# Lagrange-Labs/mapreduce-plonky2

Measured on AMD Instinct MI355X. Metric: leaf proofs/sec (whole node) + NTT GB/s vs HBM peak, 2^20-row table build, 1/2/4/8 GPU, higher is better.
Workload: dtype u64 (Goldilocks field)

## Files before the change

mapreduce-plonky2_amd/csrc/gl.cuh:

```cuda
#pragma once
#include <hip/hip_runtime.h>
#include <stdint.h>

typedef uint64_t u64;
typedef uint32_t u32;

#define GL_P 0xFFFFFFFF00000001ULL
#define GL_EPS 0xFFFFFFFFULL
#define GL_MULT_GEN 14293326489335486720ULL
#define GL_TWO_GEN 7277203076849721926ULL

#define GLD __device__ __forceinline__
#define GLHD __host__ __device__ __forceinline__

GLHD u64 gl_mk(u32 lo, u32 hi) { return ((u64)hi << 32) | lo; }
GLHD u64 gl_canon(u64 a) {
  u32 c0, c1;
  u32 t0 = __builtin_addc((u32)a, 0xFFFFFFFFu, 0u, &c0);
  u32 t1 = __builtin_addc((u32)(a >> 32), 0u, c0, &c1);
  return c1 ? gl_mk(t0, t1) : a;
}
GLHD u64 gl_add(u64 a, u64 b) {
  u32 c0, c1, d0, d1;
  u32 s0 = __builtin_addc((u32)a, (u32)b, 0u, &c0);
// ... 5 lines not shown
GLHD u64 gl_sub(u64 a, u64 b) {
  u32 c0, c1, d0, d1;
  u32 s0 = __builtin_subc((u32)a, (u32)b, 0u, &c0);
  u32 s1 = __builtin_subc((u32)(a >> 32), (u32)(b >> 32), c0, &c1);
  u32 m = c1 ? 0xFFFFFFFFu : 0u;
  u32 t0 = __builtin_subc(s0, m, 0u, &d0);
  u32 t1 = __builtin_subc(s1, 0u, d0, &d1);
  return gl_mk(t0, t1);
}
GLHD u64 gl_neg(u64 a) { return a ? GL_P - a : 0; }
GLHD u64 gl_dbl(u64 a) { return gl_add(a, a); }

GLHD u64 gl_addw(u64 a, u64 b) {
  u32 c0, c1;
  u32 s0 = __builtin_addc((u32)a, (u32)b, 0u, &c0);
  u32 s1 = __builtin_addc((u32)(a >> 32), (u32)(b >> 32), c0, &c1);
#if defined(__HIP_DEVICE_COMPILE__)
  return gl_mk(s0, s1) + (u64)(c1 ? 0xFFFFFFFFu : 0u);
#else
  u32 m = c1 ? 0xFFFFFFFFu : 0u, d0, d1;
  u32 t0 = __builtin_addc(s0, m, 0u, &d0);
  u32 t1 = __builtin_addc(s1, 0u, d0, &d1);
  return gl_mk(t0, t1);
#endif
}
GLHD u64 gl_reduce128w(u64 lo, u64 hi) {
#if defined(__HIP_DEVICE_COMPILE__)
  u32 hl = (u32)hi, hh = (u32)(hi >> 32);
  u64 t, c;
  asm("v_mad_u64_u32 %0, %1, %2, -1, %3" : "=&v"(t), "=s"(c) : "v"(hl), "v"(lo));
  u32 t0 = (u32)t, t1 = (u32)(t >> 32), r0, r1, mb, mc;
  asm("v_sub_co_u32 %0, vcc, %4, %6\n\t"
      "v_subbrev_co_u32 %1, vcc, 0, %5, vcc\n\t"
      "v_subb_co_u32 %2, vcc, %0, %0, vcc\n\t"
      "v_cndmask_b32 %3, 0, -1, %7"
      : "=&v"(r0), "=&v"(r1), "=&v"(mb), "=&v"(mc)
      : "v"(t0), "v"(t1), "v"(hh), "s"(c)
      : "vcc");
  return gl_mk(r0, r1) + gl_mk(mc - mb, mb & ~mc);
#else
  u64 hi_hi = hi >> 32, hi_lo = hi & GL_EPS;
  u64 t0;
  bool b = __builtin_sub_overflow(lo, hi_hi, &t0);
  t0 -= b ? GL_EPS : 0;
  u64 t1 = (hi_lo << 32) - hi_lo;
  u64 r;
// ... 146 lines not shown
```

mapreduce-plonky2_amd/csrc/ntt.h:

```cpp
#pragma once
#include "gl.cuh"
#include <map>
#include <memory>

namespace mp2g {

struct NttPlan {
  u32 log_n = 0, log_n1 = 0, log_n2 = 0;
  u64 *tw_a = nullptr, *tw_b = nullptr, *tw4_lo = nullptr, *tw4_hi = nullptr, *tw4_full = nullptr;
  u64 *tc_a = nullptr, *tc_b = nullptr;
  u64 n_inv = 0;
  ~NttPlan();
};
struct CosetTables {
  u32 log_n = 0, logK = 0;
  u64 shift = 0;
  u64 *lo = nullptr, *hi = nullptr, *full = nullptr;
  ~CosetTables();
};

struct NttEngine {
  hipStream_t stream = nullptr;
  std::map<u32, std::unique_ptr<NttPlan>> plans;
  std::map<u64, std::unique_ptr<CosetTables>> cosets;
  u64* scratch = nullptr;
  size_t scratch_words = 0;
  u64 generation = 0;
  ~NttEngine();

  hipError_t plan(u32 log_n, bool inverse, NttPlan** out);
  hipError_t coset(u32 log_n, u32 logK, u64 shift, CosetTables** out);
  hipError_t ensure_scratch(size_t words);
  hipError_t run(const u64* in, u64* out, u32 log_n, u32 polys, u32 logK, u64 in_poly_stride,
                 u64 out_poly_stride, bool inverse, const CosetTables* pre, bool bitrev_out);
// ... 6 lines not shown
```

mapreduce-plonky2_amd/csrc/ntt.hip:

```cpp
#include "ntt.h"
#include <cstdlib>

namespace mp2g {

__device__ __forceinline__ int lds_pad(int a) { return a + (a >> 4); }

struct NttArgs {
  const u64* in;
  u64* out;
  u64 in_poly_stride, out_poly_stride;
  u32 logK;
  u32 log_n, log_n1, log_n2;
  u32 batch;
  const u64* tw;
  const u64* tw4_lo;
  const u64* tw4_hi;
  const u64* pre_lo;
  const u64* pre_hi;
  const u64* tw4_full;
  const u64* pre_full;
  u64 post;
  u32 bitrev_out;
  u32 inverse;
  const u64* tc;
};

template <int LT, int LW> struct NttGeom {
  static constexpr int E = (1 << LT) << LW;
  static constexpr int NT = (E >> 3) < 64 ? 64 : ((E >> 3) > 1024 ? 1024 : (E >> 3));
};
template <int LT> struct R8Tw {
  static constexpr int lo(int rho) { return LT - 3 - 3 * rho; }
  static constexpr int n_tables() { int r = 0; while (lo(r) >= 1) r++; return r; }
  static constexpr int off(int rho) { int o = 0; for (int q = 0; q < rho; q++) o += 7 << lo(q); return o; }
  static constexpr int TOTAL = off(n_tables());
  static constexpr int GLOBAL_ROUNDS = (LT >= 11 && n_tables() >= 1) ? 1 : 0;
  static constexpr int LDS_OFF = off(GLOBAL_ROUNDS);
  static constexpr int LDS_WORDS = TOTAL - LDS_OFF;
};
__device__ __forceinline__ u64 gl_mul_2p24(u64 x) { return gl_canon(gl_reduce96w(x << 24, x >> 40)); }
__device__ __forceinline__ u64 gl_mul_2p48(u64 x) { return gl_reduce128(x << 48, x >> 16); }
__device__ __forceinline__ u64 gl_mul_2p72(u64 x) {
  return gl_sub(gl_reduce128(0, x << 8), (x >> 56) << 32);
}
template <int K> __device__ __forceinline__ u64 gl_mul_w8(u64 x) {
  return K == 1 ? gl_mul_2p24(x) : (K == 2 ? gl_mul_2p48(x) : gl_mul_2p72(x));
}
__device__ __forceinline__ u64 gl_sub_mul_2p48(u64 u, u64 v) {
  u32 c0, c1;
  const u32 s0 = __builtin_subc((u32)u, (u32)v, 0u, &c0);
  const u32 s1 = __builtin_subc((u32)(u >> 32), (u32)(v >> 32), c0, &c1);
  const u64 s = gl_mk(s0, s1);
  return gl_reduce128(gl_mk(c1 ? 0x10000u : 0u, s0 << 16), s >> 16);
}
__device__ __forceinline__ u64 gl_sub_mul_2p72(u64 u, u64 v) {
  u32 c0, c1;
  const u32 s0 = __builtin_subc((u32)u, (u32)v, 0u, &c0);
  const u32 s1 = __builtin_subc((u32)(u >> 32), (u32)(v >> 32), c0, &c1);
  const u64 s = gl_mk(s0, s1);
  return gl_sub(gl_reduce128(gl_mk(0u, c1 ? 0x100u : 0u), s << 8), (s >> 56) << 32);
}
template <int K> __device__ __forceinline__ u64 gl_sub_mul_w8(u64 u, u64 v) {
  return K == 1 ? gl_mul_2p24(gl_sub(u, v)) : (K == 2 ? gl_sub_mul_2p48(u, v) : gl_sub_mul_2p72(u, v));
}
template <int K> __device__ __forceinline__ u64 bfly_lo(u64 u, u64 v, bool inverse) {
  return inverse ? gl_sub_mul_w8<4 - K>(v, u) : gl_sub_mul_w8<K>(u, v);
}
template <int S> __device__ __forceinline__ u64 gl_mul_2pow(u64 x) {
  static_assert(S >= 0 && S < 192, "exponent mod 192");
  if constexpr (S == 0) return x;
  else if constexpr (S >= 96) return gl_neg(gl_mul_2pow<S - 96>(x));
  else if constexpr (S <= 32) return gl_canon(gl_reduce96w(x << S, x >> (64 - S)));
  else if constexpr (S < 64) return gl_reduce128(x << S, x >> (64 - S));
  else if constexpr (S == 64) return gl_reduce128(0, x);
  else {
    constexpr int K = S - 64;
    return gl_sub(gl_reduce128(0, x << K), (x >> (64 - K)) << 32);
  }
}
template <int A, bool INV, int M> __device__ __forceinline__ u64 shift_tw1(u64 x) {
  constexpr int R = ((M & 1) << 2) | (M & 2) | (M >> 2);
  constexpr int E = (A * R) & 63;
  return gl_mul_2pow<3 * (INV ? (64 - E) & 63 : E)>(x);
}
template <int A, bool INV> __device__ __forceinline__ void shift_tw(u64* x) {
  x[1] = shift_tw1<A, INV, 1>(x[1]); x[2] = shift_tw1<A, INV, 2>(x[2]); x[3] = shift_tw1<A, INV, 3>(x[3]); x[4] = shift_tw1<A, INV, 4>(x[4]);
  x[5] = shift_tw1<A, INV, 5>(x[5]); x[6] = shift_tw1<A, INV, 6>(x[6]); x[7] = shift_tw1<A, INV, 7>(x[7]);
}
template <bool INV> __device__ __forceinline__ void shift_twiddles_dir(u64* x, int a) {
  switch (a) {
    case 1: shift_tw<1, INV>(x); break;
    case 2: shift_tw<2, INV>(x); break;
    case 3: shift_tw<3, INV>(x); break;
    case 4: shift_tw<4, INV>(x); break;
    case 5: shift_tw<5, INV>(x); break;
    case 6: shift_tw<6, INV>(x); break;
    case 7: shift_tw<7, INV>(x); break;
    default: break;
  }
}
__device__ __forceinline__ void shift_twiddles(u64* x, int a, bool inverse) {
  if (inverse) shift_twiddles_dir<true>(x, a); else shift_twiddles_dir<false>(x, a);
}

template <int LT, int HI, int R, bool TWG = false, bool MERGED = false>
__device__ __forceinline__ void butterfly(u64* x, int below, const u64* tw, const u64* __restrict__ twg, bool inverse) {
  constexpr int LO = HI - R + 1;
  constexpr int RHO = (LT - 1 - HI) / 3;
  static_assert(R == 3 || LO == 0, "a partial round can only be the last one");
  if constexpr (R == 3) {
    { u64 u = x[0], v = x[4]; x[0] = gl_add(u, v); x[4] = gl_sub(u, v); }
    { u64 u = x[1], v = x[5]; x[1] = gl_add(u, v); x[5] = bfly_lo<1>(u, v, inverse); }
    { u64 u = x[2], v = x[6]; x[2] = gl_add(u, v); x[6] = bfly_lo<2>(u, v, inverse); }
    { u64 u = x[3], v = x[7]; x[3] = gl_add(u, v); x[7] = bfly_lo<3>(u, v, inverse); }
#pragma unroll
    for (int h = 0; h < 8; h += 4) {
      { u64 u = x[h], v = x[h + 2]; x[h] = gl_add(u, v); x[h + 2] = gl_sub(u, v); }
      { u64 u = x[h + 1], v = x[h + 3]; x[h + 1] = gl_add(u, v); x[h + 3] = bfly_lo<2>(u, v, inverse); }
    }
#pragma unroll
    for (int m = 0; m < 8; m += 2) {
      u64 u = x[m], v = x[m + 1];
      x[m] = (MERGED || (LO > 1 && m > 0)) ? gl_addw(u, v) : gl_add(u, v);
      x[m + 1] = gl_sub(u, v);
    }
    if constexpr (MERGED) {
#pragma unroll
      for (int m = 0; m < 8; m++) {
        const int r = ((m & 1) << 2) | (m & 2) | (m >> 2);
        x[m] = gl_mul(x[m], twg[((8 * r) << LO) + below]);
      }
    } else if constexpr (LO == 1) {
      if (inverse) {
        x[1] = below ? gl_mul_2pow<192 - 48>(x[1]) : x[1]; x[2] = below ? gl_mul_2pow<192 - 24>(x[2]) : x[2]; x[3] = below ? gl_mul_2pow<192 - 72>(x[3]) : x[3];
        x[4] = below ? gl_mul_2pow<192 - 12>(x[4]) : x[4]; x[5] = below ? gl_mul_2pow<192 - 60>(x[5]) : x[5]; x[6] = below ? gl_mul_2pow<192 - 36>(x[6]) : x[6];
        x[7] = below ? gl_mul_2pow<192 - 84>(x[7]) : x[7];
      } else {
        x[1] = below ? gl_mul_2pow<48>(x[1]) : x[1]; x[2] = below ? gl_mul_2pow<24>(x[2]) : x[2]; x[3] = below ? gl_mul_2pow<72>(x[3]) : x[3];
        x[4] = below ? gl_mul_2pow<12>(x[4]) : x[4]; x[5] = below ? gl_mul_2pow<60>(x[5]) : x[5]; x[6] = below ? gl_mul_2pow<36>(x[6]) : x[6];
        x[7] = below ? gl_mul_2pow<84>(x[7]) : x[7];
      }
    } else if constexpr (LO > 0) {
      const u64* tab = (TWG || RHO < R8Tw<LT>::GLOBAL_ROUNDS) ? twg + R8Tw<LT>::off(RHO) : tw + (R8Tw<LT>::off(RHO) - R8Tw<LT>::LDS_OFF);
#pragma unroll
      for (int m = 1; m < 8; m++) {
        const int r = ((m & 1) << 2) | (m & 2) | (m >> 2);
        x[m] = gl_mul(x[m], tab[((r - 1) << LO) + below]);
      }
    }
  } else if constexpr (R == 2) {
    { u64 u = x[0], v = x[2]; x[0] = gl_add(u, v); x[2] = gl_sub(u, v); }
    { u64 u = x[1], v = x[3]; x[1] = gl_add(u, v); x[3] = bfly_lo<2>(u, v, inverse); }
    { u64 u = x[0], v = x[1]; x[0] = gl_add(u, v); x[1] = gl_sub(u, v); }
    { u64 u = x[2], v = x[3]; x[2] = gl_add(u, v); x[3] = gl_sub(u, v); }
  } else {
    u64 u = x[0], v = x[1]; x[0] = gl_add(u, v); x[1] = gl_sub(u, v);
  }
}
template <int LT, int HI, int R, bool COLS, int LW, int NTT_THREADS>
__device__ __forceinline__ void dif_round(u64* s, const u64* tw, const u64* __restrict__ twg, int tid, bool inverse) {
  constexpr int T = 1 << LT, LO = HI - R + 1, W = 1 << LW;
  constexpr int ITEMS = W << (LT - R);
  for (int item = tid; item < ITEMS; item += NTT_THREADS) {
    int c, rest;
    if (COLS) { c = item & (W - 1); rest = item >> LW; }
    else { rest = item & ((T >> R) - 1); c = item >> (LT - R); }
    int below = rest & ((1 << LO) - 1), above = rest >> LO;
    int j0 = (above << (HI + 1)) | below;
    u64 x[1 << R];
#pragma unroll
    for (int m = 0; m < (1 << R); m++) {
      int j = j0 + (m << LO);
      x[m] = s[lds_pad(COLS ? (j << LW) + c : (c << LT) + j)];
    }
    butterfly<LT, HI, R>(x, below, tw, twg, inverse);
#pragma unroll
    for (int m = 0; m < (1 << R); m++) {
      int j = j0 + (m << LO);
      s[lds_pad(COLS ? (j << LW) + c : (c << LT) + j)] = x[m];
// ... 21 lines not shown

template <int LT, int LW>
__global__ void __launch_bounds__((NttGeom<LT, LW>::NT)) ntt_rows_kernel(NttArgs a) {
  constexpr int T = 1 << LT, E = T << LW, NT = NttGeom<LT, LW>::NT;
  extern __shared__ __align__(16) u64 smem[];
  u64* s = smem;
  u64* tw = smem + lds_pad(E) + 1;
  const int tid = threadIdx.x;
  for (int i = tid; i < R8Tw<LT>::LDS_WORDS; i += NT) tw[i] = a.tw[R8Tw<LT>::LDS_OFF + i];
  const u32 n1 = 1u << a.log_n1;
  const u64 total_rows = (u64)a.batch << a.log_n1;
  const u64 row0 = (u64)blockIdx.x << LW;
  const bool two_pass = a.log_n1 != 0;
  for (int e = tid; e < E; e += NT) {
    int r = e >> LT, j = e & (T - 1);
    u64 g = row0 + r;
    u64 v = 0;
    if (g < total_rows) {
      u32 b = (u32)(g >> a.log_n1), jr = (u32)(g & (n1 - 1));
      if (two_pass) {
        v = out_base(a, b)[((u64)jr << LT) + j];
      } else {
        v = in_base(a, b)[j];
        if (a.pre_lo) v = gl_mul(v, a.pre_lo[((u64)(b & ((1u << a.logK) - 1)) << LT) + j]);
      }
    }
    s[lds_pad(e)] = v;
  }
  __syncthreads();
  dif_all<LT, LT - 1, false, LW, NT>(s, tw, a.tw, tid, a.inverse != 0);
  for (int e = tid; e < E; e += NT) {
    int r = e >> LT, p = e & (T - 1);
    u64 g = row0 + r;
    if (g >= total_rows) continue;
    u32 b = (u32)(g >> a.log_n1), jr = (u32)(g & (n1 - 1));
    u64 v = a.bitrev_out ? s[lds_pad(e)] : s[lds_pad((r << LT) + (int)bitrev32((u32)p, LT))];
    if (a.post) v = gl_mul(v, a.post);
    out_base(a, b)[((u64)jr << LT) + p] = v;
  }
}
template <int LT, int LW>
__global__ void __launch_bounds__((NttGeom<LT, LW>::NT)) ntt_rows_nat_kernel(NttArgs a) {
  constexpr int T = 1 << LT, W = 1 << LW, E = T << LW, NT = NttGeom<LT, LW>::NT;
  extern __shared__ __align__(16) u64 smem[];
  u64* s = smem;
  u64* tw = smem + lds_pad(E) + 1;
  const int tid = threadIdx.x;
  for (int i = tid; i < R8Tw<LT>::LDS_WORDS; i += NT) tw[i] = a.tw[R8Tw<LT>::LDS_OFF + i];
  const u32 lo_bits = a.log_n1 - LW;
  const u32 tile = blockIdx.x;
  const u32 b = tile >> lo_bits, jr_lo = tile & ((1u << lo_bits) - 1);
  const u64* src = a.in + (u64)b * ((u64)1 << a.log_n);
  for (int e = tid; e < E; e += NT) {
    u32 jr = ((u32)(e >> LT) << lo_bits) | jr_lo;
    s[lds_pad(e)] = src[((u64)jr << LT) + (e & (T - 1))];
  }
  __syncthreads();
  dif_all<LT, LT - 1, false, LW, NT>(s, tw, a.tw, tid, a.inverse != 0);
  u64* dst = out_base(a, b);
  const u32 k1_hi = bitrev32(jr_lo, lo_bits) << LW;
  for (int e = tid; e < E; e += NT) {
    int q = e & (W - 1), k2 = e >> LW;
    int row = (int)bitrev32((u32)q, LW);
    u64 v = s[lds_pad((row << LT) + (int)bitrev32((u32)k2, LT))];
    if (a.post) v = gl_mul(v, a.post);
    dst[(u64)(k1_hi | (u32)q) + ((u64)k2 << a.log_n1)] = v;
  }
}

template <int LT, int LW>
__global__ void __launch_bounds__((NttGeom<LT, LW>::NT)) ntt_cols_kernel(NttArgs a, u64* dst_dense) {
  constexpr int T = 1 << LT, W = 1 << LW, E = T << LW, NT = NttGeom<LT, LW>::NT;
  extern __shared__ __align__(16) u64 smem[];
  u64* s = smem;
  u64* tw = smem + lds_pad(E) + 1;
  const int tid = threadIdx.x;
  for (int i = tid; i < R8Tw<LT>::LDS_WORDS; i += NT) tw[i] = a.tw[R8Tw<LT>::LDS_OFF + i];
  const u32 tiles_per = 1u << (a.log_n2 - LW);
  u32 bid = blockIdx.x;
  if ((gridDim.x & 7) == 0) bid = (bid & 7) * (gridDim.x >> 3) + (bid >> 3);
  const u32 b = bid / tiles_per, c0 = (bid % tiles_per) << LW;
  const u32 coset = b & ((1u << a.logK) - 1);
  const u64* src = in_base(a, b);
  for (int e = tid; e < E; e += NT) {
    int c = e & (W - 1), j = e >> LW;
    u64 v = src[((u64)j << a.log_n2) + c0 + c];
    if (a.pre_full) {
      v = gl_mul(v, a.pre_full[((u64)coset << a.log_n) + ((u64)j << a.log_n2) + c0 + c]);
    } else if (a.pre_lo) {
      v = gl_mul(v, a.pre_lo[((u64)coset << a.log_n2) + c0 + c]);
      v = gl_mul(v, a.pre_hi[((u64)coset << LT) + j]);
    }
    s[lds_pad(e)] = v;
  }
  __syncthreads();
  dif_all<LT, LT - 1, true, LW, NT>(s, tw, a.tw, tid, a.inverse != 0);
  u64* dst = dst_dense ? dst_dense + (u64)b * ((u64)1 << a.log_n) : out_base(a, b);
  for (int e = tid; e < E; e += NT) {
    int c = e & (W - 1), j = e >> LW;
    u64 v = s[lds_pad(e)];
    u64 w;
    if (a.tw4_full) {
      w = a.tw4_full[((u64)j << a.log_n2) + c0 + c];
    } else {
      u32 k1 = bitrev32((u32)j, LT);
      u32 ex = (c0 + c) * k1;
      w = gl_mul(a.tw4_lo[ex & 4095], a.tw4_hi[ex >> 12]);
    }
    dst[((u64)j << a.log_n2) + c0 + c] = gl_mul(v, w);
  }
}

template <int LT, int LW, bool COLS> struct WaveGeom {
  static constexpr int NBR = LT > 12 ? 2 : 1;
  static constexpr int LTS = LT - 3 * NBR;
  static constexpr int LWL = 9 - LTS;
  static constexpr bool OK = LT >= 3 && LT <= 13 && (!COLS || LT <= 12) && ((1 << LT) << LW) == 8 * NttGeom<LT, LW>::NT && (!COLS || LW >= LWL);
};
template <int LT, int LW, bool COLS> struct ShiftGeom {
  using G = WaveGeom<LT, LW, COLS>;
  static constexpr int L0 = LT - 3;
  static constexpr bool OK = G::OK && G::NBR == 1 && G::LTS >= 6 && (COLS ? (LW + L0 - 3 >= 6) : (LW == 0 && L0 - 3 >= 6));
  static constexpr int TC_WORDS = 64 << (L0 - 3);
};
__device__ __forceinline__ void wave_sync() {
  __builtin_amdgcn_fence(__ATOMIC_RELEASE, "wavefront");
  __builtin_amdgcn_wave_barrier();
  __builtin_amdgcn_fence(__ATOMIC_ACQUIRE, "wavefront");
}
template <int LT, int LTS, int HI, int R, bool COLS, int LWL, int LWS, bool MERGED = false>
__device__ __forceinline__ void wave_round(u64* s, int base, const u64* tw, int lane, bool inverse, const u64* __restrict__ tcw = nullptr) {
  constexpr int LO = HI - R + 1, WL = 1 << LWL;
// ... 41 lines not shown
  const int tid = threadIdx.x, lane = tid & 63, wave = tid >> 6;
  for (int i = tid; i < R8Tw<LT>::LDS_WORDS; i += NT) tw[i] = a.tw[R8Tw<LT>::LDS_OFF + i];
  const u32 n1 = 1u << a.log_n1;
  const u64 total_rows = (u64)a.batch << a.log_n1;
  const u64 row0 = (u64)blockIdx.x << LW;
  const bool two_pass = a.log_n1 != 0, inverse = a.inverse != 0;
  {
    const int c = tid >> L0, below = tid & ((1 << L0) - 1);
    const u64 g = row0 + c;
    u64 x[8];
    if (g < total_rows) {
      u32 b = (u32)(g >> a.log_n1), jr = (u32)(g & (n1 - 1));
      if (two_pass) {
        const u64* src = out_base(a, b) + ((u64)jr << LT);
#pragma unroll
        for (int m = 0; m < 8; m++) x[m] = src[below + (m << L0)];
      } else {
        const u64* src = in_base(a, b);
#pragma unroll
        for (int m = 0; m < 8; m++) x[m] = src[below + (m << L0)];
        if (a.pre_lo) {
          const u64* pre = a.pre_lo + ((u64)(b & ((1u << a.logK) - 1)) << LT);
#pragma unroll
          for (int m = 0; m < 8; m++) x[m] = gl_mul(x[m], pre[below + (m << L0)]);
        }
      }
    } else {
#pragma unroll
      for (int m = 0; m < 8; m++) x[m] = 0;
    }
    if constexpr (SHIFT) {
      butterfly<LT, 2, 3>(x, 0, nullptr, nullptr, inverse);
      shift_twiddles(x, __builtin_amdgcn_readfirstlane(below >> (L0 - 3)), inverse);
    } else {
      butterfly<LT, LT - 1, 3, true>(x, below, tw, a.tw, inverse);
    }
#pragma unroll
    for (int m = 0; m < 8; m++) s[lds_pad((c << LT) + below + (m << L0))] = x[m];
  }
  __syncthreads();
  if constexpr (G::NBR == 2) {
    dif_round<LT, LT - 4, 3, false, LW, NT>(s, tw, a.tw, tid, inverse);
    __syncthreads();
  }
  if constexpr (SHIFT) {
    const int r = __builtin_amdgcn_readfirstlane((int)bitrev32((u32)(wave & 7), 3));
    wave_rounds<LT, LTS, LTS - 1, false, G::LWL, 0, true>(s, wave << 9, tw, lane, inverse, a.tc + (r << (L0 - 3)));
  } else {
    wave_rounds<LT, LTS, LTS - 1, false, G::LWL, 0>(s, wave << 9, tw, lane, inverse);
  }
  if (a.bitrev_out) {
    wave_sync();
    u64 v[8];
#pragma unroll
    for (int k = 0; k < 8; k++) v[k] = s[lds_pad((wave << 9) + lane + (k << 6))];
    if (a.post) {
#pragma unroll
      for (int k = 0; k < 8; k++) v[k] = gl_mul(v[k], a.post);
    }
#pragma unroll
    for (int k = 0; k < 8; k++) {
      int e = (wave << 9) + lane + (k << 6);
      int r = e >> LT, p = e & (T - 1);
      u64 g = row0 + r;
      if (g >= total_rows) continue;
      u32 b = (u32)(g >> a.log_n1), jr = (u32)(g & (n1 - 1));
      out_base(a, b)[((u64)jr << LT) + p] = v[k];
    }
  } else {
    __syncthreads();
    for (int e = tid; e < E; e += NT) {
      int r = e >> LT, p = e & (T - 1);
      u64 g = row0 + r;
      if (g >= total_rows) continue;
      u32 b = (u32)(g >> a.log_n1), jr = (u32)(g & (n1 - 1));
      u64 v = s[lds_pad((r << LT) + (int)bitrev32((u32)p, LT))];
      if (a.post) v = gl_mul(v, a.post);
      out_base(a, b)[((u64)jr << LT) + p] = v;
    }
  }
}

template <int LT, int LW, bool SHIFT = false>
__global__ void __launch_bounds__((NttGeom<LT, LW>::NT)) __attribute__((amdgpu_waves_per_eu(8))) ntt_cols_v2_kernel(NttArgs a, u64* dst_dense) {
  using G = WaveGeom<LT, LW, true>;
  static_assert(!SHIFT || ShiftGeom<LT, LW, true>::OK, "tile shape without wave-uniform shift twiddles");
  constexpr int W = 1 << LW, E = (1 << LT) << LW, NT = NttGeom<LT, LW>::NT, LTS = G::LTS, LWL = G::LWL;
  extern __shared__ __align__(16) u64 smem[];
  u64* s = smem;
  u64* tw = smem + lds_pad(E) + 1;
  const int tid = threadIdx.x, lane = tid & 63, wave = tid >> 6;
  for (int i = tid; i < R8Tw<LT>::LDS_WORDS; i += NT) tw[i] = a.tw[R8Tw<LT>::LDS_OFF + i];
  const u32 tiles_per = 1u << (a.log_n2 - LW);
  u32 bid = blockIdx.x;
  if ((gridDim.x & 7) == 0) bid = (bid & 7) * (gridDim.x >> 3) + (bid >> 3);
  const u32 b = bid / tiles_per, c0 = (bid % tiles_per) << LW;
  const u32 coset = b & ((1u << a.logK) - 1);
  const u64* src = in_base(a, b);
  const bool inverse = a.inverse != 0;
  {
    const int c = tid & (W - 1), below = tid >> LW;
    u64 x[8];
#pragma unroll
    for (int m = 0; m < 8; m++) x[m] = src[((u64)(below + (m << LTS)) << a.log_n2) + c0 + c];
    if (a.pre_full) {
      const u64* pre = a.pre_full + ((u64)coset << a.log_n) + c0 + c;
#pragma unroll
      for (int m = 0; m < 8; m++) x[m] = gl_mul(x[m], pre[(u64)(below + (m << LTS)) << a.log_n2]);
    } else if (a.pre_lo) {
      u64 pl = a.pre_lo[((u64)coset << a.log_n2) + c0 + c];
#pragma unroll
      for (int m = 0; m < 8; m++) x[m] = gl_mul(gl_mul(x[m], pl), a.pre_hi[((u64)coset << LT) + below + (m << LTS)]);
    }
    if constexpr (SHIFT) {
      butterfly<LT, 2, 3>(x, 0, nullptr, nullptr, inverse);
      shift_twiddles(x, __builtin_amdgcn_readfirstlane(below >> (LTS - 3)), inverse);
    } else {
      butterfly<LT, LT - 1, 3, true>(x, below, tw, a.tw, inverse);
    }
#pragma unroll
    for (int m = 0; m < 8; m++) s[lds_pad(((below + (m << LTS)) << LW) + c)] = x[m];
  }
  __syncthreads();
  {
    constexpr int GW = W >> LWL;
    const int cg = wave & (GW - 1), jh = wave / GW;
    if constexpr (SHIFT) {
      const int r = __builtin_amdgcn_readfirstlane((int)bitrev32((u32)jh, 3));
      wave_rounds<LT, LTS, LTS - 1, true, LWL, LW, true>(s, ((jh << LTS) << LW) + (cg << LWL), tw, lane, inverse, a.tc + (r << (LTS - 3)));
    } else {
      wave_rounds<LT, LTS, LTS - 1, true, LWL, LW>(s, ((jh << LTS) << LW) + (cg << LWL), tw, lane, inverse);
    }
  }
  __syncthreads();
  u64* dst = dst_dense ? dst_dense + (u64)b * ((u64)1 << a.log_n) : out_base(a, b);
#pragma unroll
  for (int k = 0; k < 8; k++) {
    int e = tid + k * NT;
    int c = e & (W - 1), j = e >> LW;
    u64 v = s[lds_pad(e)];
    u64 w;
    if (a.tw4_full) {
      w = a.tw4_full[((u64)j << a.log_n2) + c0 + c];
    } else {
      u32 k1 = bitrev32((u32)j, LT);
      u32 ex = (c0 + c) * k1;
      w = gl_mul(a.tw4_lo[ex & 4095], a.tw4_hi[ex >> 12]);
    }
    dst[((u64)j << a.log_n2) + c0 + c] = gl_mul(v, w);
  }
}

__global__ void r8_round_twiddles_kernel(u64* out, u64 w, u32 lo, u32 shift) {
  u32 i = blockIdx.x * blockDim.x + threadIdx.x;
  if (i >= (7u << lo)) return;
  u32 r = (i >> lo) + 1, below = i & ((1u << lo) - 1);
  out[i] = gl_pow(w, ((u64)below << shift) * r);
}
__global__ void merged_twiddles_kernel(u64* out, u64 w, u32 lb) {
  u32 i = blockIdx.x * blockDim.x + threadIdx.x;
  if (i >= (64u << lb)) return;
  out[i] = gl_pow(w, (u64)(i & ((1u << lb) - 1)) * (i >> lb));
}
__global__ void powers_kernel(u64* out, u64 base, u64 first, u64 stride_exp, u32 count) {
  u32 i = blockIdx.x * blockDim.x + threadIdx.x;
  if (i >= count) return;
  out[i] = gl_mul(first, gl_pow(base, (u64)i * stride_exp));
}
__global__ void coset_tables_kernel(u64* lo, u64* hi, u64 shift, u64 w_nk, u32 log_n1, u32 log_n2, u32 K) {
  u32 i = blockIdx.x * blockDim.x + threadIdx.x;
  u32 n1 = 1u << log_n1, n2 = 1u << log_n2;
  u32 per = n1 + n2;
  if (i >= per * K) return;
  u32 j = i / per, r = i % per;
  u64 sj = gl_mul(shift, gl_pow(w_nk, j));
  if (r < n2) lo[(u64)j * n2 + r] = gl_pow(sj, r);
  else hi[(u64)j * n1 + (r - n2)] = gl_pow(sj, (u64)(r - n2) << log_n2);
}
__global__ void tw4_full_kernel(u64* out, u64 wn, u32 log_n1, u32 log_n2) {
  u64 i = (u64)blockIdx.x * blockDim.x + threadIdx.x;
  if (i >= ((u64)1 << (log_n1 + log_n2))) return;
  u32 j = (u32)(i >> log_n2), i2 = (u32)(i & ((1u << log_n2) - 1));
  out[i] = gl_pow(wn, (u64)i2 * bitrev32(j, log_n1));
}
__global__ void pre_full_kernel(u64* out, u64 shift, u64 w_nk, u32 log_n, u32 K) {
  u64 i = (u64)blockIdx.x * blockDim.x + threadIdx.x;
  if (i >= ((u64)K << log_n)) return;
  u32 c = (u32)(i >> log_n);
  out[i] = gl_pow(gl_mul(shift, gl_pow(w_nk, c)), i & (((u64)1 << log_n) - 1));
}
__global__ void scale_powers_kernel(u64* data, u32 log_n, u32 batch, u64 base, u64 first) {
  u64 i = (u64)blockIdx.x * blockDim.x + threadIdx.x;
  if (i >= ((u64)batch << log_n)) return;
  u64 k = i & (((u64)1 << log_n) - 1);
  data[i] = gl_mul(data[i], gl_mul(first, gl_pow(base, k)));
}
__global__ void scale_table_kernel(u64* __restrict__ data, u32 log_n, u32 batch, const u64* __restrict__ table) {
  u64 i = (u64)blockIdx.x * blockDim.x + threadIdx.x;
  if (i >= ((u64)batch << log_n)) return;
  data[i] = gl_mul(data[i], table[i & (((u64)1 << log_n) - 1)]);
}

#define HIPCHK(x) do { hipError_t e_ = (x); if (e_ != hipSuccess) return e_; } while (0)

static hipError_t dev_alloc(u64** p, size_t words) { return hipMalloc((void**)p, words * sizeof(u64)); }

// ... 9 lines not shown
  if (log_n >= 22) l1 = log_n - 12;
  return l1;
}
template <int LT> static constexpr int rows_lw() { return LT >= 12 ? 0 : (LT == 11 ? 2 : 12 - LT); }
template <int LT> static constexpr int cols_lw() { return LT >= 11 ? 2 : (LT == 10 ? 3 : 12 - LT); }
template <int LT> static constexpr bool shift_rows_lt() { return ShiftGeom<LT, rows_lw<LT>(), false>::OK; }
template <int LT> static constexpr bool shift_cols_lt() { return ShiftGeom<LT, cols_lw<LT>(), true>::OK; }
static bool shift_rows_ok(u32 lt) {
  switch (lt) { case 12: return shift_rows_lt<12>(); case 13: return shift_rows_lt<13>(); default: return false; }
}
static bool shift_cols_ok(u32 lt) {
  switch (lt) { case 9: return shift_cols_lt<9>(); case 10: return shift_cols_lt<10>(); case 11: return shift_cols_lt<11>(); case 12: return shift_cols_lt<12>(); default: return false; }
}
hipError_t NttEngine::plan(u32 log_n, bool inverse, NttPlan** out) {
  u32 key = log_n * 2 + (inverse ? 1 : 0);
  auto it = plans.find(key);
  if (it != plans.end()) { *out = it->second.get(); return hipSuccess; }
  std::unique_ptr<NttPlan> p(new NttPlan());
  p->log_n = log_n;
  p->log_n1 = split_log_n1(log_n);
  p->log_n2 = log_n - p->log_n1;
  u64 wn = gl_root_of_unity(log_n);
  if (inverse) wn = gl_inv(wn);
  auto powers = [&](u64** dst, u64 base, u32 count) -> hipError_t {
    HIPCHK(dev_alloc(dst, count ? count : 1));
    if (count) hipLaunchKernelGGL(powers_kernel, dim3((count + 255) / 256), dim3(256), 0, stream, *dst, base, (u64)1, (u64)1, count);
    return hipGetLastError();
  };
  u64 w2 = gl_pow(wn, (u64)1 << p->log_n1), w1 = gl_pow(wn, (u64)1 << p->log_n2);
  auto stage_tw = [&](u64** dst, u64 base, u32 lt) -> hipError_t {
    HIPCHK(dev_alloc(dst, (size_t)1 << lt));
    u32 off = 0;
    for (u32 rho = 0; (int)lt - 3 - 3 * (int)rho >= 1; rho++) {
      u32 lo = lt - 3 - 3 * rho, count = 7u << lo;
      hipLaunchKernelGGL(r8_round_twiddles_kernel, dim3((count + 255) / 256), dim3(256), 0, stream, *dst + off, base, lo, 3 * rho);
      HIPCHK(hipGetLastError());
      off += count;
    }
    return hipSuccess;
  };
  auto merged_tw = [&](u64** dst, u64 base, u32 lt) -> hipError_t {
    const u32 lb = lt - 6, count = 64u << lb;
    HIPCHK(dev_alloc(dst, count));
    hipLaunchKernelGGL(merged_twiddles_kernel, dim3((count + 255) / 256), dim3(256), 0, stream, *dst, base, lb);
    return hipGetLastError();
  };
  HIPCHK(stage_tw(&p->tw_b, w2, p->log_n2));
  if (shift_rows_ok(p->log_n2)) HIPCHK(merged_tw(&p->tc_b, w2, p->log_n2));
  if (p->log_n1) {
    HIPCHK(stage_tw(&p->tw_a, w1, p->log_n1));
    if (shift_cols_ok(p->log_n1)) HIPCHK(merged_tw(&p->tc_a, w1, p->log_n1));
    HIPCHK(powers(&p->tw4_lo, wn, 4096));
    HIPCHK(powers(&p->tw4_hi, gl_pow(wn, 4096), log_n > 12 ? (1u << (log_n - 12)) : 1));
    if (log_n <= 22) {
      HIPCHK(dev_alloc(&p->tw4_full, (size_t)1 << log_n));
      hipLaunchKernelGGL(tw4_full_kernel, dim3((u32)((((u64)1 << log_n) + 255) / 256)), dim3(256), 0, stream, p->tw4_full, wn, p->log_n1, p->log_n2);
      HIPCHK(hipGetLastError());
    }
  }
  p->n_inv = inverse ? gl_inv(((u64)1 << log_n) % GL_P) : 0;
  *out = p.get();
  plans[key] = std::move(p);
  return hipSuccess;
}

hipError_t NttEngine::coset(u32 log_n, u32 logK, u64 shift, CosetTables** out) {
  u64 key = ((u64)log_n << 8 | logK) ^ (shift * 0x9E3779B97F4A7C15ULL);
  auto it = cosets.find(key);
  if (it != cosets.end() && it->second->shift == shift && it->second->log_n == log_n && it->second->logK == logK) {
    *out = it->second.get(); return hipSuccess;
  }
  std::unique_ptr<CosetTables> c(new CosetTables());
  c->log_n = log_n; c->logK = logK; c->shift = shift;
  u32 log_n1 = split_log_n1(log_n), log_n2 = log_n - log_n1;
  u32 K = 1u << logK, n1 = 1u << log_n1, n2 = 1u << log_n2;
  HIPCHK(dev_alloc(&c->lo, (size_t)K * n2));
  HIPCHK(dev_alloc(&c->hi, (size_t)K * n1));
  u32 total = (n1 + n2) * K;
  hipLaunchKernelGGL(coset_tables_kernel, dim3((total + 255) / 256), dim3(256), 0, stream, c->lo, c->hi, shift,
                     gl_root_of_unity(log_n + logK), log_n1, log_n2, K);
  HIPCHK(hipGetLastError());
  if (log_n1 && ((u64)K << log_n) <= ((u64)1 << 23)) {
    HIPCHK(dev_alloc(&c->full, (size_t)K << log_n));
// ... 106 lines not shown
    default: return hipErrorInvalidValue;
  }
}
#define COLS_CASE(N) case N: return launch_cols<N, cols_lw<N>()>(a, dense, st);
static hipError_t dispatch_cols(u32 lt, const NttArgs& a, u64* dense, hipStream_t st) {
  switch (lt) {
    COLS_CASE(7) COLS_CASE(8) COLS_CASE(9) COLS_CASE(10) COLS_CASE(11) COLS_CASE(12)
    default: return hipErrorInvalidValue;
  }
}

hipError_t NttEngine::run(const u64* in, u64* out, u32 log_n, u32 polys, u32 logK, u64 in_poly_stride,
                          u64 out_poly_stride, bool inverse, const CosetTables* pre, bool bitrev_out) {
  if (log_n == 0 || log_n > 24) return hipErrorInvalidValue;
  NttPlan* p;
  HIPCHK(plan(log_n, inverse, &p));
  NttArgs a{};
  a.in = in; a.out = out;
  a.in_poly_stride = in_poly_stride; a.out_poly_stride = out_poly_stride;
  a.logK = logK; a.log_n = log_n; a.log_n1 = p->log_n1; a.log_n2 = p->log_n2;
  a.batch = polys << logK;
  a.tw4_lo = p->tw4_lo; a.tw4_hi = p->tw4_hi; a.tw4_full = p->tw4_full;
  a.pre_lo = pre ? pre->lo : nullptr; a.pre_hi = pre ? pre->hi : nullptr; a.pre_full = pre ? pre->full : nullptr;
  a.post = p->n_inv;
  a.bitrev_out = bitrev_out ? 1 : 0;
  a.inverse = inverse ? 1 : 0;
  if (p->log_n1 == 0) {
    a.tw = p->tw_b; a.tc = p->tc_b;
    return dispatch_rows(p->log_n2, a, false, stream);
  }
  u64* dense = nullptr;
  if (!bitrev_out) {
    HIPCHK(ensure_scratch((size_t)a.batch << log_n));
    dense = scratch;
  }
  a.tw = p->tw_a; a.tc = p->tc_a;
  HIPCHK(dispatch_cols(p->log_n1, a, dense, stream));
  a.tw = p->tw_b; a.tc = p->tc_b;
  a.pre_lo = a.pre_hi = a.pre_full = nullptr;
  if (!bitrev_out) a.in = dense;
  return dispatch_rows(p->log_n2, a, !bitrev_out, stream);
}

hipError_t NttEngine::scale_powers(u64* data, u32 log_n, u32 batch, u64 base, u64 first) {
  u64 total = (u64)batch << log_n;
  hipLaunchKernelGGL(scale_powers_kernel, dim3((u32)((total + 255) / 256)), dim3(256), 0, stream, data, log_n, batch, base, first);
  return hipGetLastError();
// ... 11 lines not shown
```

Before: 931.9.

## Use lazy non-canonical Goldilocks arithmetic in NTT butterflies and fold n^-1 into twiddles

Butterflies, twiddle multiplies and pre-scaling now use new inline-asm add/sub/neg helpers and weak (non-canonical) reductions. Canonicalisation happens once at the final store. The inverse-NTT scaling by n^-1 is folded into the precomputed twiddle tables (tw4_lo, tw4_full, merged tc_b) or done as a shift-based multiply by 2^-k instead of a full field multiply per element. The aim is fewer ALU instructions per butterfly and per output. The cost is more complex correctness invariants around partially reduced values and plan-dependent scaling logic.

```diff
diff --git a/mapreduce-plonky2_amd/csrc/gl.cuh b/mapreduce-plonky2_amd/csrc/gl.cuh
--- a/mapreduce-plonky2_amd/csrc/gl.cuh
+++ b/mapreduce-plonky2_amd/csrc/gl.cuh
@@ -51,6 +51,93 @@
   u32 t0 = __builtin_addc(s0, m, 0u, &d0);
   u32 t1 = __builtin_addc(s1, 0u, d0, &d1);
   return gl_mk(t0, t1);
+#endif
+}
+GLHD u64 gl_add_ww(u64 a, u64 b) {
+#if defined(__HIP_DEVICE_COMPILE__)
+  u32 r0, r1, m;
+  asm("v_add_co_u32 %0, vcc, %3, %5\n\t"
+      "v_addc_co_u32 %1, vcc, %4, %6, vcc\n\t"
+      "v_subb_co_u32 %2, vcc, %0, %0, vcc\n\t"
+      "v_add_co_u32 %0, vcc, %0, %2\n\t"
+      "v_addc_co_u32 %1, vcc, 0, %1, vcc\n\t"
+      "v_subb_co_u32 %2, vcc, %2, %2, vcc"
+      : "=&v"(r0), "=v"(r1), "=v"(m)
+      : "v"((u32)a), "v"((u32)(a >> 32)), "v"((u32)b), "v"((u32)(b >> 32))
+      : "vcc");
+  return gl_mk(r0, r1) + (u64)m;
+#else
+  u64 s, r;
+  bool c = __builtin_add_overflow(a, b, &s);
+  bool c2 = __builtin_add_overflow(s, c ? GL_EPS : 0, &r);
+  return r + (c2 ? GL_EPS : 0);
+#endif
+}
+GLHD u64 gl_sub_ww(u64 a, u64 b) {
+#if defined(__HIP_DEVICE_COMPILE__)
+  u32 r0, r1, m;
+  asm("v_sub_co_u32 %0, vcc, %3, %5\n\t"
+      "v_subb_co_u32 %1, vcc, %4, %6, vcc\n\t"
+      "v_subb_co_u32 %2, vcc, %0, %0, vcc\n\t"
+      "v_sub_co_u32 %0, vcc, %0, %2\n\t"
+      "v_subbrev_co_u32 %1, vcc, 0, %1, vcc\n\t"
+      "v_subb_co_u32 %2, vcc, %2, %2, vcc"
+      : "=&v"(r0), "=v"(r1), "=v"(m)
+      : "v"((u32)a), "v"((u32)(a >> 32)), "v"((u32)b), "v"((u32)(b >> 32))
+      : "vcc");
+  return gl_mk(r0, r1) + gl_mk(0u - m, m);
+#else
+  u64 d, r;
+  bool c = __builtin_sub_overflow(a, b, &d);
+  bool c2 = __builtin_sub_overflow(d, c ? GL_EPS : 0, &r);
+  return r - (c2 ? GL_EPS : 0);
+#endif
+}
+GLHD u64 gl_sub_borrow(u64 a, u64 b, u32& m) {
+#if defined(__HIP_DEVICE_COMPILE__)
+  u32 r0, r1;
+  asm("v_sub_co_u32 %0, vcc, %3, %5\n\t"
+      "v_subb_co_u32 %1, vcc, %4, %6, vcc\n\t"
+      "v_subb_co_u32 %2, vcc, %0, %0, vcc"
+      : "=&v"(r0), "=v"(r1), "=v"(m)
+      : "v"((u32)a), "v"((u32)(a >> 32)), "v"((u32)b), "v"((u32)(b >> 32))
+      : "vcc");
+  return gl_mk(r0, r1);
+#else
+  u64 d;
+  m = __builtin_sub_overflow(a, b, &d) ? 0xFFFFFFFFu : 0u;
+  return d;
+#endif
+}
+GLHD u64 gl_negw(u64 a) {
+#if defined(__HIP_DEVICE_COMPILE__)
+  u32 r0, r1, m;
+  asm("v_sub_co_u32 %0, vcc, 1, %3\n\t"
+      "v_subb_co_u32 %1, vcc, -1, %4, vcc\n\t"
+      "v_subb_co_u32 %2, vcc, %0, %0, vcc"
+      : "=&v"(r0), "=v"(r1), "=v"(m)
+      : "v"((u32)a), "v"((u32)(a >> 32))
+      : "vcc");
+  return gl_mk(r0, r1) + gl_mk(0u - m, m);
+#else
+  u32 m;
+  const u64 r = gl_sub_borrow(GL_P, a, m);
+  return r + gl_mk(0u - m, m);
+#endif
+}
+GLHD u64 gl_canon_vcc(u64 a) {
+#if defined(__HIP_DEVICE_COMPILE__)
+  u32 t0, t1;
+  asm("v_add_co_u32 %0, vcc, -1, %2\n\t"
+      "v_addc_co_u32 %1, vcc, 0, %3, vcc\n\t"
+      "v_cndmask_b32 %0, %2, %0, vcc\n\t"
+      "v_cndmask_b32 %1, %3, %1, vcc"
+      : "=&v"(t0), "=&v"(t1)
+      : "v"((u32)a), "v"((u32)(a >> 32))
+      : "vcc");
+  return gl_mk(t0, t1);
+#else
+  return gl_canon(a);
 #endif
 }
 GLHD u64 gl_reduce128w(u64 lo, u64 hi) {
diff --git a/mapreduce-plonky2_amd/csrc/ntt.h b/mapreduce-plonky2_amd/csrc/ntt.h
--- a/mapreduce-plonky2_amd/csrc/ntt.h
+++ b/mapreduce-plonky2_amd/csrc/ntt.h
@@ -9,7 +9,7 @@
   u32 log_n = 0, log_n1 = 0, log_n2 = 0;
   u64 *tw_a = nullptr, *tw_b = nullptr, *tw4_lo = nullptr, *tw4_hi = nullptr, *tw4_full = nullptr;
   u64 *tc_a = nullptr, *tc_b = nullptr;
-  u64 n_inv = 0;
+  bool ninv_in_tc = false;
   ~NttPlan();
 };
 struct CosetTables {
diff --git a/mapreduce-plonky2_amd/csrc/ntt.hip b/mapreduce-plonky2_amd/csrc/ntt.hip
--- a/mapreduce-plonky2_amd/csrc/ntt.hip
+++ b/mapreduce-plonky2_amd/csrc/ntt.hip
@@ -1,4 +1,5 @@
 #include "ntt.h"
+#include "ntt_shift.cuh"
 #include <cstdlib>
 
 namespace mp2g {
@@ -19,7 +20,7 @@
   const u64* pre_hi;
   const u64* tw4_full;
   const u64* pre_full;
-  u64 post;
+  u32 post_k;
   u32 bitrev_out;
   u32 inverse;
   const u64* tc;
@@ -38,45 +39,8 @@
   static constexpr int LDS_OFF = off(GLOBAL_ROUNDS);
   static constexpr int LDS_WORDS = TOTAL - LDS_OFF;
 };
-__device__ __forceinline__ u64 gl_mul_2p24(u64 x) { return gl_canon(gl_reduce96w(x << 24, x >> 40)); }
-__device__ __forceinline__ u64 gl_mul_2p48(u64 x) { return gl_reduce128(x << 48, x >> 16); }
-__device__ __forceinline__ u64 gl_mul_2p72(u64 x) {
-  return gl_sub(gl_reduce128(0, x << 8), (x >> 56) << 32);
-}
-template <int K> __device__ __forceinline__ u64 gl_mul_w8(u64 x) {
-  return K == 1 ? gl_mul_2p24(x) : (K == 2 ? gl_mul_2p48(x) : gl_mul_2p72(x));
-}
-__device__ __forceinline__ u64 gl_sub_mul_2p48(u64 u, u64 v) {
-  u32 c0, c1;
-  const u32 s0 = __builtin_subc((u32)u, (u32)v, 0u, &c0);
-  const u32 s1 = __builtin_subc((u32)(u >> 32), (u32)(v >> 32), c0, &c1);
-  const u64 s = gl_mk(s0, s1);
-  return gl_reduce128(gl_mk(c1 ? 0x10000u : 0u, s0 << 16), s >> 16);
-}
-__device__ __forceinline__ u64 gl_sub_mul_2p72(u64 u, u64 v) {
-  u32 c0, c1;
-  const u32 s0 = __builtin_subc((u32)u, (u32)v, 0u, &c0);
-  const u32 s1 = __builtin_subc((u32)(u >> 32), (u32)(v >> 32), c0, &c1);
-  const u64 s = gl_mk(s0, s1);
-  return gl_sub(gl_reduce128(gl_mk(0u, c1 ? 0x100u : 0u), s << 8), (s >> 56) << 32);
-}
-template <int K> __device__ __forceinline__ u64 gl_sub_mul_w8(u64 u, u64 v) {
-  return K == 1 ? gl_mul_2p24(gl_sub(u, v)) : (K == 2 ? gl_sub_mul_2p48(u, v) : gl_sub_mul_2p72(u, v));
-}
 template <int K> __device__ __forceinline__ u64 bfly_lo(u64 u, u64 v, bool inverse) {
   return inverse ? gl_sub_mul_w8<4 - K>(v, u) : gl_sub_mul_w8<K>(u, v);
-}
-template <int S> __device__ __forceinline__ u64 gl_mul_2pow(u64 x) {
-  static_assert(S >= 0 && S < 192, "exponent mod 192");
-  if constexpr (S == 0) return x;
-  else if constexpr (S >= 96) return gl_neg(gl_mul_2pow<S - 96>(x));
-  else if constexpr (S <= 32) return gl_canon(gl_reduce96w(x << S, x >> (64 - S)));
-  else if constexpr (S < 64) return gl_reduce128(x << S, x >> (64 - S));
-  else if constexpr (S == 64) return gl_reduce128(0, x);
-  else {
-    constexpr int K = S - 64;
-    return gl_sub(gl_reduce128(0, x << K), (x >> (64 - K)) << 32);
-  }
 }
 template <int A, bool INV, int M> __device__ __forceinline__ u64 shift_tw1(u64 x) {
   constexpr int R = ((M & 1) << 2) | (M & 2) | (M >> 2);
@@ -109,26 +73,26 @@
   constexpr int RHO = (LT - 1 - HI) / 3;
   static_assert(R == 3 || LO == 0, "a partial round can only be the last one");
   if constexpr (R == 3) {
-    { u64 u = x[0], v = x[4]; x[0] = gl_add(u, v); x[4] = gl_sub(u, v); }
-    { u64 u = x[1], v = x[5]; x[1] = gl_add(u, v); x[5] = bfly_lo<1>(u, v, inverse); }
-    { u64 u = x[2], v = x[6]; x[2] = gl_add(u, v); x[6] = bfly_lo<2>(u, v, inverse); }
-    { u64 u = x[3], v = x[7]; x[3] = gl_add(u, v); x[7] = bfly_lo<3>(u, v, inverse); }
+    { u64 u = x[0], v = x[4]; x[0] = gl_add_ww(u, v); x[4] = gl_sub_ww(u, v); }
+    { u64 u = x[1], v = x[5]; x[1] = gl_add_ww(u, v); x[5] = bfly_lo<1>(u, v, inverse); }
+    { u64 u = x[2], v = x[6]; x[2] = gl_add_ww(u, v); x[6] = bfly_lo<2>(u, v, inverse); }
+    { u64 u = x[3], v = x[7]; x[3] = gl_add_ww(u, v); x[7] = bfly_lo<3>(u, v, inverse); }
 #pragma unroll
     for (int h = 0; h < 8; h += 4) {
-      { u64 u = x[h], v = x[h + 2]; x[h] = gl_add(u, v); x[h + 2] = gl_sub(u, v); }
-      { u64 u = x[h + 1], v = x[h + 3]; x[h + 1] = gl_add(u, v); x[h + 3] = bfly_lo<2>(u, v, inverse); }
+      { u64 u = x[h], v = x[h + 2]; x[h] = gl_add_ww(u, v); x[h + 2] = gl_sub_ww(u, v); }
+      { u64 u = x[h + 1], v = x[h + 3]; x[h + 1] = gl_add_ww(u, v); x[h + 3] = bfly_lo<2>(u, v, inverse); }
     }
 #pragma unroll
     for (int m = 0; m < 8; m += 2) {
       u64 u = x[m], v = x[m + 1];
-      x[m] = (MERGED || (LO > 1 && m > 0)) ? gl_addw(u, v) : gl_add(u, v);
-      x[m + 1] = gl_sub(u, v);
+      x[m] = gl_add_ww(u, v);
+      x[m + 1] = gl_sub_ww(u, v);
     }
     if constexpr (MERGED) {
 #pragma unroll
       for (int m = 0; m < 8; m++) {
         const int r = ((m & 1) << 2) | (m & 2) | (m >> 2);
-        x[m] = gl_mul(x[m], twg[((8 * r) << LO) + below]);
+        x[m] = gl_mulw(x[m], twg[((8 * r) << LO) + below]);
       }
     } else if constexpr (LO == 1) {
       if (inverse) {
@@ -145,16 +109,16 @@
 #pragma unroll
       for (int m = 1; m < 8; m++) {
         const int r = ((m & 1) << 2) | (m & 2) | (m >> 2);
-        x[m] = gl_mul(x[m], tab[((r - 1) << LO) + below]);
+        x[m] = gl_mulw(x[m], tab[((r - 1) << LO) + below]);
       }
     }
   } else if constexpr (R == 2) {
-    { u64 u = x[0], v = x[2]; x[0] = gl_add(u, v); x[2] = gl_sub(u, v); }
-    { u64 u = x[1], v = x[3]; x[1] = gl_add(u, v); x[3] = bfly_lo<2>(u, v, inverse); }
-    { u64 u = x[0], v = x[1]; x[0] = gl_add(u, v); x[1] = gl_sub(u, v); }
-    { u64 u = x[2], v = x[3]; x[2] = gl_add(u, v); x[3] = gl_sub(u, v); }
+    { u64 u = x[0], v = x[2]; x[0] = gl_add_ww(u, v); x[2] = gl_sub_ww(u, v); }
+    { u64 u = x[1], v = x[3]; x[1] = gl_add_ww(u, v); x[3] = bfly_lo<2>(u, v, inverse); }
+    { u64 u = x[0], v = x[1]; x[0] = gl_add_ww(u, v); x[1] = gl_sub_ww(u, v); }
+    { u64 u = x[2], v = x[3]; x[2] = gl_add_ww(u, v); x[3] = gl_sub_ww(u, v); }
   } else {
-    u64 u = x[0], v = x[1]; x[0] = gl_add(u, v); x[1] = gl_sub(u, v);
+    u64 u = x[0], v = x[1]; x[0] = gl_add_ww(u, v); x[1] = gl_sub_ww(u, v);
   }
 }
 template <int LT, int HI, int R, bool COLS, int LW, int NTT_THREADS>
@@ -222,7 +186,7 @@
         v = out_base(a, b)[((u64)jr << LT) + j];
       } else {
         v = in_base(a, b)[j];
-        if (a.pre_lo) v = gl_mul(v, a.pre_lo[((u64)(b & ((1u << a.logK) - 1)) << LT) + j]);
+        if (a.pre_lo) v = gl_mulw(v, a.pre_lo[((u64)(b & ((1u << a.logK) - 1)) << LT) + j]);
       }
     }
     s[lds_pad(e)] = v;
@@ -235,8 +199,8 @@
     if (g >= total_rows) continue;
     u32 b = (u32)(g >> a.log_n1), jr = (u32)(g & (n1 - 1));
     u64 v = a.bitrev_out ? s[lds_pad(e)] : s[lds_pad((r << LT) + (int)bitrev32((u32)p, LT))];
-    if (a.post) v = gl_mul(v, a.post);
-    out_base(a, b)[((u64)jr << LT) + p] = v;
+    if (a.post_k) v = gl_mul_inv_2pow(v, a.post_k);
+    out_base(a, b)[((u64)jr << LT) + p] = gl_canon_vcc(v);
   }
 }
 template <int LT, int LW>
@@ -263,8 +227,8 @@
     int q = e & (W - 1), k2 = e >> LW;
     int row = (int)bitrev32((u32)q, LW);
     u64 v = s[lds_pad((row << LT) + (int)bitrev32((u32)k2, LT))];
-    if (a.post) v = gl_mul(v, a.post);
-    dst[(u64)(k1_hi | (u32)q) + ((u64)k2 << a.log_n1)] = v;
+    if (a.post_k) v = gl_mul_inv_2pow(v, a.post_k);
+    dst[(u64)(k1_hi | (u32)q) + ((u64)k2 << a.log_n1)] = gl_canon_vcc(v);
   }
 }
 
@@ -286,10 +250,10 @@
     int c = e & (W - 1), j = e >> LW;
     u64 v = src[((u64)j << a.log_n2) + c0 + c];
     if (a.pre_full) {
-      v = gl_mul(v, a.pre_full[((u64)coset << a.log_n) + ((u64)j << a.log_n2) + c0 + c]);
+      v = gl_mulw(v, a.pre_full[((u64)coset << a.log_n) + ((u64)j << a.log_n2) + c0 + c]);
     } else if (a.pre_lo) {
-      v = gl_mul(v, a.pre_lo[((u64)coset << a.log_n2) + c0 + c]);
-      v = gl_mul(v, a.pre_hi[((u64)coset << LT) + j]);
+      v = gl_mulw(v, a.pre_lo[((u64)coset << a.log_n2) + c0 + c]);
+      v = gl_mulw(v, a.pre_hi[((u64)coset << LT) + j]);
     }
     s[lds_pad(e)] = v;
   }
@@ -305,9 +269,9 @@
     } else {
       u32 k1 = bitrev32((u32)j, LT);
       u32 ex = (c0 + c) * k1;
-      w = gl_mul(a.tw4_lo[ex & 4095], a.tw4_hi[ex >> 12]);
-    }
-    dst[((u64)j << a.log_n2) + c0 + c] = gl_mul(v, w);
+      w = gl_mulw(a.tw4_lo[ex & 4095], a.tw4_hi[ex >> 12]);
+    }
+    dst[((u64)j << a.log_n2) + c0 + c] = gl_canon_vcc(gl_mulw(v, w));
   }
 }
 
@@ -395,7 +359,7 @@
         if (a.pre_lo) {
           const u64* pre = a.pre_lo + ((u64)(b & ((1u << a.logK) - 1)) << LT);
 #pragma unroll
-          for (int m = 0; m < 8; m++) x[m] = gl_mul(x[m], pre[below + (m << L0)]);
+          for (int m = 0; m < 8; m++) x[m] = gl_mulw(x[m], pre[below + (m << L0)]);
         }
       }
     } else {
@@ -427,10 +391,12 @@
     u64 v[8];
 #pragma unroll
     for (int k = 0; k < 8; k++) v[k] = s[lds_pad((wave << 9) + lane + (k << 6))];
-    if (a.post) {
-#pragma unroll
-      for (int k = 0; k < 8; k++) v[k] = gl_mul(v[k], a.post);
-    }
+    if (a.post_k) {
+#pragma unroll
+      for (int k = 0; k < 8; k++) v[k] = gl_mul_inv_2pow(v[k], a.post_k);
+    }
+#pragma unroll
+    for (int k = 0; k < 8; k++) v[k] = gl_canon_vcc(v[k]);
 #pragma unroll
     for (int k = 0; k < 8; k++) {
       int e = (wave << 9) + lane + (k << 6);
@@ -448,8 +414,8 @@
       if (g >= total_rows) continue;
       u32 b = (u32)(g >> a.log_n1), jr = (u32)(g & (n1 - 1));
       u64 v = s[lds_pad((r << LT) + (int)bitrev32((u32)p, LT))];
-      if (a.post) v = gl_mul(v, a.post);
-      out_base(a, b)[((u64)jr << LT) + p] = v;
+      if (a.post_k) v = gl_mul_inv_2pow(v, a.post_k);
+      out_base(a, b)[((u64)jr << LT) + p] = gl_canon_vcc(v);
     }
   }
 }
@@ -479,11 +445,11 @@
     if (a.pre_full) {
       const u64* pre = a.pre_full + ((u64)coset << a.log_n) + c0 + c;
 #pragma unroll
-      for (int m = 0; m < 8; m++) x[m] = gl_mul(x[m], pre[(u64)(below + (m << LTS)) << a.log_n2]);
+      for (int m = 0; m < 8; m++) x[m] = gl_mulw(x[m], pre[(u64)(below + (m << LTS)) << a.log_n2]);
     } else if (a.pre_lo) {
       u64 pl = a.pre_lo[((u64)coset << a.log_n2) + c0 + c];
 #pragma unroll
-      for (int m = 0; m < 8; m++) x[m] = gl_mul(gl_mul(x[m], pl), a.pre_hi[((u64)coset << LT) + below + (m << LTS)]);
+      for (int m = 0; m < 8; m++) x[m] = gl_mulw(gl_mulw(x[m], pl), a.pre_hi[((u64)coset << LT) + below + (m << LTS)]);
     }
     if constexpr (SHIFT) {
       butterfly<LT, 2, 3>(x, 0, nullptr, nullptr, inverse);
@@ -518,9 +484,9 @@
     } else {
       u32 k1 = bitrev32((u32)j, LT);
       u32 ex = (c0 + c) * k1;
-      w = gl_mul(a.tw4_lo[ex & 4095], a.tw4_hi[ex >> 12]);
-    }
-    dst[((u64)j << a.log_n2) + c0 + c] = gl_mul(v, w);
+      w = gl_mulw(a.tw4_lo[ex & 4095], a.tw4_hi[ex >> 12]);
+    }
+    dst[((u64)j << a.log_n2) + c0 + c] = gl_canon_vcc(gl_mulw(v, w));
   }
 }
 
@@ -530,10 +496,10 @@
   u32 r = (i >> lo) + 1, below = i & ((1u << lo) - 1);
   out[i] = gl_pow(w, ((u64)below << shift) * r);
 }
-__global__ void merged_twiddles_kernel(u64* out, u64 w, u32 lb) {
+__global__ void merged_twiddles_kernel(u64* out, u64 w, u32 lb, u64 first) {
   u32 i = blockIdx.x * blockDim.x + threadIdx.x;
   if (i >= (64u << lb)) return;
-  out[i] = gl_pow(w, (u64)(i & ((1u << lb) - 1)) * (i >> lb));
+  out[i] = gl_mul(first, gl_pow(w, (u64)(i & ((1u << lb) - 1)) * (i >> lb)));
 }
 __global__ void powers_kernel(u64* out, u64 base, u64 first, u64 stride_exp, u32 count) {
   u32 i = blockIdx.x * blockDim.x + threadIdx.x;
@@ -550,11 +516,11 @@
   if (r < n2) lo[(u64)j * n2 + r] = gl_pow(sj, r);
   else hi[(u64)j * n1 + (r - n2)] = gl_pow(sj, (u64)(r - n2) << log_n2);
 }
-__global__ void tw4_full_kernel(u64* out, u64 wn, u32 log_n1, u32 log_n2) {
+__global__ void tw4_full_kernel(u64* out, u64 wn, u32 log_n1, u32 log_n2, u64 first) {
   u64 i = (u64)blockIdx.x * blockDim.x + threadIdx.x;
   if (i >= ((u64)1 << (log_n1 + log_n2))) return;
   u32 j = (u32)(i >> log_n2), i2 = (u32)(i & ((1u << log_n2) - 1));
-  out[i] = gl_pow(wn, (u64)i2 * bitrev32(j, log_n1));
+  out[i] = gl_mul(first, gl_pow(wn, (u64)i2 * bitrev32(j, log_n1)));
 }
 __global__ void pre_full_kernel(u64* out, u64 shift, u64 w_nk, u32 log_n, u32 K) {
   u64 i = (u64)blockIdx.x * blockDim.x + threadIdx.x;
@@ -610,9 +576,10 @@
   p->log_n2 = log_n - p->log_n1;
   u64 wn = gl_root_of_unity(log_n);
   if (inverse) wn = gl_inv(wn);
-  auto powers = [&](u64** dst, u64 base, u32 count) -> hipError_t {
+  const u64 n_inv = inverse ? gl_inv(((u64)1 << log_n) % GL_P) : 1;
+  auto powers = [&](u64** dst, u64 base, u64 first, u32 count) -> hipError_t {
     HIPCHK(dev_alloc(dst, count ? count : 1));
-    if (count) hipLaunchKernelGGL(powers_kernel, dim3((count + 255) / 256), dim3(256), 0, stream, *dst, base, (u64)1, (u64)1, count);
+    if (count) hipLaunchKernelGGL(powers_kernel, dim3((count + 255) / 256), dim3(256), 0, stream, *dst, base, first, (u64)1, count);
     return hipGetLastError();
   };
   u64 w2 = gl_pow(wn, (u64)1 << p->log_n1), w1 = gl_pow(wn, (u64)1 << p->log_n2);
@@ -627,26 +594,26 @@
     }
     return hipSuccess;
   };
-  auto merged_tw = [&](u64** dst, u64 base, u32 lt) -> hipError_t {
+  auto merged_tw = [&](u64** dst, u64 base, u32 lt, u64 first) -> hipError_t {
     const u32 lb = lt - 6, count = 64u << lb;
     HIPCHK(dev_alloc(dst, count));
-    hipLaunchKernelGGL(merged_twiddles_kernel, dim3((count + 255) / 256), dim3(256), 0, stream, *dst, base, lb);
+    hipLaunchKernelGGL(merged_twiddles_kernel, dim3((count + 255) / 256), dim3(256), 0, stream, *dst, base, lb, first);
     return hipGetLastError();
   };
   HIPCHK(stage_tw(&p->tw_b, w2, p->log_n2));
-  if (shift_rows_ok(p->log_n2)) HIPCHK(merged_tw(&p->tc_b, w2, p->log_n2));
+  p->ninv_in_tc = inverse && p->log_n1 == 0 && shift_rows_ok(p->log_n2);
+  if (shift_rows_ok(p->log_n2)) HIPCHK(merged_tw(&p->tc_b, w2, p->log_n2, p->ninv_in_tc ? n_inv : 1));
   if (p->log_n1) {
     HIPCHK(stage_tw(&p->tw_a, w1, p->log_n1));
-    if (shift_cols_ok(p->log_n1)) HIPCHK(merged_tw(&p->tc_a, w1, p->log_n1));
-    HIPCHK(powers(&p->tw4_lo, wn, 4096));
-    HIPCHK(powers(&p->tw4_hi, gl_pow(wn, 4096), log_n > 12 ? (1u << (log_n - 12)) : 1));
+    if (shift_cols_ok(p->log_n1)) HIPCHK(merged_tw(&p->tc_a, w1, p->log_n1, 1));
+    HIPCHK(powers(&p->tw4_lo, wn, n_inv, 4096));
+    HIPCHK(powers(&p->tw4_hi, gl_pow(wn, 4096), 1, log_n > 12 ? (1u << (log_n - 12)) : 1));
     if (log_n <= 22) {
       HIPCHK(dev_alloc(&p->tw4_full, (size_t)1 << log_n));
-      hipLaunchKernelGGL(tw4_full_kernel, dim3((u32)((((u64)1 << log_n) + 255) / 256)), dim3(256), 0, stream, p->tw4_full, wn, p->log_n1, p->log_n2);
+      hipLaunchKernelGGL(tw4_full_kernel, dim3((u32)((((u64)1 << log_n) + 255) / 256)), dim3(256), 0, stream, p->tw4_full, wn, p->log_n1, p->log_n2, n_inv);
       HIPCHK(hipGetLastError());
     }
   }
-  p->n_inv = inverse ? gl_inv(((u64)1 << log_n) % GL_P) : 0;
   *out = p.get();
   plans[key] = std::move(p);
   return hipSuccess;
@@ -799,7 +766,7 @@
   a.batch = polys << logK;
   a.tw4_lo = p->tw4_lo; a.tw4_hi = p->tw4_hi; a.tw4_full = p->tw4_full;
   a.pre_lo = pre ? pre->lo : nullptr; a.pre_hi = pre ? pre->hi : nullptr; a.pre_full = pre ? pre->full : nullptr;
-  a.post = p->n_inv;
+  a.post_k = inverse && p->log_n1 == 0 && !(p->ninv_in_tc && !use_v1()) ? log_n : 0;
   a.bitrev_out = bitrev_out ? 1 : 0;
   a.inverse = inverse ? 1 : 0;
   if (p->log_n1 == 0) {
diff --git a/mapreduce-plonky2_amd/csrc/ntt_shift.cuh b/mapreduce-plonky2_amd/csrc/ntt_shift.cuh
--- /dev/null
+++ b/mapreduce-plonky2_amd/csrc/ntt_shift.cuh
@@ -0,0 +1,34 @@
+#pragma once
+#include "gl.cuh"
+
+template <int S> GLHD u64 gl_mul_2pow(u64 x) {
+  static_assert(S >= 0 && S < 192, "exponent mod 192");
+  if constexpr (S == 0) return x;
+  else if constexpr (S >= 96) return gl_negw(gl_mul_2pow<S - 96>(x));
+  else if constexpr (S <= 32) return gl_reduce96w(x << S, x >> (64 - S));
+  else if constexpr (S < 64) return gl_reduce128w(x << S, x >> (64 - S));
+  else if constexpr (S == 64) return gl_reduce128w(0, x);
+  else {
+    constexpr int K = S - 64;
+    return gl_reduce128w(gl_mk(1u, ~(u32)(x >> (64 - K))), x << K);
+  }
+}
+template <int K> GLHD u64 gl_mul_w8(u64 x) { return gl_mul_2pow<24 * K>(x); }
+GLHD u64 gl_sub_mul_2p48(u64 u, u64 v) {
+  u32 m;
+  const u64 s = gl_sub_borrow(u, v, m);
+  return gl_reduce128w(gl_mk(m & 0x10000u, (u32)s << 16), s >> 16);
+}
+GLHD u64 gl_sub_mul_2p72(u64 u, u64 v) {
+  u32 m;
+  const u64 s = gl_sub_borrow(u, v, m);
+  return gl_reduce128w(gl_mk(1u + m, ~((u32)(s >> 56) - (m & 0x101u))), s << 8);
+}
+template <int K> GLHD u64 gl_sub_mul_w8(u64 u, u64 v) {
+  if constexpr (K == 1) return gl_mul_2pow<24>(gl_sub_ww(u, v));
+  else if constexpr (K == 2) return gl_sub_mul_2p48(u, v);
+  else return gl_sub_mul_2p72(u, v);
+}
+GLHD u64 gl_mul_inv_2pow(u64 x, u32 k) {
+  return gl_negw(gl_reduce128w(gl_mk(1u, ~(u32)(x >> (32 + k))), x << (32 - k)));
+}
```

After: 924.4. No clear change (-0.8%).
